# OmerShubi/DL_VQA

Measured on AMD Instinct MI355X. Metric: VQA samples/sec (train step), higher is better.
Workload: dtype f32; 1 GPU; VqaNet train step (fwd+softCE+bwd+Adam), batch 256/GPU, 224x224 images, 14-token questions, 1000-way head, train mode; global_batch=256, image_size=224, answers=1000, vocab=5000, parallelism=dp1

## Files before the change

dl_vqa_amd/_lib.py:

```python
from __future__ import annotations

import ctypes as C
import os

import torch

_HERE = os.path.dirname(os.path.abspath(__file__))
LIB_PATH = os.environ.get("VQA_LIB", os.path.join(_HERE, "libvqa_hip.so"))
HEADER_PATH = os.path.join(os.path.dirname(_HERE), "include", "vqa_hip.h")


def header_abi_version() -> int:
    import re
    with open(HEADER_PATH) as f:
        m = re.search(r"^#define\s+VQA_ABI_VERSION\s+(\d+)", f.read(), flags=re.M)
    if not m:
        raise VqaHipError(f"{HEADER_PATH}: no VQA_ABI_VERSION")
    return int(m.group(1))


f32p = C.c_void_p
u8p = C.c_void_p
i64p = C.c_void_p
i32, i64, f32, u64, vp = C.c_int, C.c_int64, C.c_float, C.c_uint64, C.c_void_p
# ... 96 lines not shown
    "vqa_gemm_tall_bf16_supported": (i32, [i32, i32, i32, i32, i32]),
    "vqa_gemm_tall_bf16_plan": (i32, [i32, i32, i32, C.POINTER(i32), i32]),
    "vqa_gemm_tall_bf16": (i32, [vp, i64, vp, i64, vp, i64, i32, i32, i32, f32p, i64, i32, i32, i32, i32, vp]),
    "vqa_conv_pack_weights_bf16": (i32, [f32p, vp, vp, i32, i32, i32, vp]),
    "vqa_conv3x3_relu_pool_fwd_bf16": (i32, [vp, vp, f32p, vp, i32, u8p, i32, i32, i32, i32, i32, i32, i32, vp]),
    "vqa_conv3x3_dgrad_bf16": (i32, [vp, u8p, vp, vp, i32, i32, i32, i32, i32, i32, i32, i32, vp]),
    "vqa_conv3x3_wgrad_bf16_workspace_bytes": (i64, [i32, i32, i32, i32, i32, i32]),
    "vqa_conv3x3_wgrad_bf16": (i32, [vp, vp, u8p, f32p, f32p, i32, i32, i32, i32, i32, i32, i32, f32p, i64, i32, vp]),
    "vqa_pconvf_supported": (i32, [i32, i32, i32, i32, i32]),
    "vqa_pconvf_weights_bytes": (i64, [i32, i32]),
    "vqa_pconvf_pack_weights": (i32, [f32p, f32p, i32, i32, vp]),
    "vqa_pconvf_dgrad": (i32, [f32p, u8p, f32p, f32p, i32, i32, i32, i32, i32, i32, vp]),
    "vqa_pconv_supported": (i32, [i32, i32, i32, i32, i32]),
    "vqa_pconv_weights_bytes": (i64, [i32, i32]),
    "vqa_pconv_pack_weights": (i32, [f32p, vp, vp, i32, i32, vp]),
    "vqa_pconv_fwd": (i32, [vp, vp, f32p, vp, i32, u8p, i32, i32, i32, i32, i32, i32, vp]),
    "vqa_pconv_wgrad_supported": (i32, [i32, i32, i32, i32]),
    "vqa_pconv_wgrad_workspace_bytes": (i64, [i32, i32, i32, i32, i32]),
    "vqa_pconv_wgrad": (i32, [vp, u8p, vp, f32p, f32p, i32, i32, i32, i32, i32, f32p, i64, i32, vp]),
    "vqa_pconv_dgrad": (i32, [vp, u8p, vp, vp, i32, i32, i32, i32, i32, i32, i32, vp]),
    "vqa_adam": (i32, [f32p, f32p, f32p, f32p, i64, f32, f32, f32, f32, i32, f32, vp]),
    "vqa_adam_segments": (i32, [f32p, f32p, f32p, f32p, i64, vp, i32, f32, vp]),
    "vqa_conv3x3_x3_plan": (i32, [i32, i32, i32, i32, i32, i32, i32, C.POINTER(i32), i32]),
}

K_GEMM, K_CONV_FWD, K_CONV_DGRAD, K_CONV_WGRAD = 0, 1, 2, 3
(K_L2NORM_FWD, K_L2NORM_BWD, K_ATT_SCORE_FWD, K_ATT_SCORE_BWD, K_ATT_APPLY_FWD, K_ATT_APPLY_BWD, K_ADAM, K_SOFTCE,
 K_DROPOUT, K_LSTM_SEQ, K_COUNT) = range(4, 15)


class LstmDir(C.Structure):
    _fields_ = [("w_hh", vp), ("xg", vp), ("gates", vp), ("Hs", vp), ("Cs", vp), ("c_final", vp),
                ("dgates", vp), ("dh", vp), ("dc", vp), ("reverse", i32)]


class AdamSegment(C.Structure):
    _fields_ = [("begin", i64), ("end", i64), ("lr", f32), ("beta1", f32), ("beta2", f32), ("eps", f32),
                ("weight_decay", f32), ("step", i32), ("decoupled", i32)]


ADAM_MAX_SEGMENTS = 64


class VqaHipError(RuntimeError):
    pass


_lib = None


def load() -> C.CDLL:
    global _lib
    if _lib is not None:
        return _lib
    if not os.path.exists(LIB_PATH):
        raise VqaHipError(
            f"{LIB_PATH} not found: build it with `python -m dl_vqa_amd.build` "
            "(the HIP extension is mandatory; there is no CPU fallback)")
    lib = C.CDLL(LIB_PATH)
    for name, (res, args) in PROTOTYPES.items():
        fn = getattr(lib, name)
        fn.restype = res
        fn.argtypes = args
    want = header_abi_version()
# ... 21 lines not shown
```

dl_vqa_amd/build.py:

```python
from __future__ import annotations

import os
import subprocess
import sys
from concurrent.futures import ThreadPoolExecutor

HERE = os.path.dirname(os.path.abspath(__file__))
CSRC = os.path.join(HERE, "csrc")
LIB = os.path.join(HERE, "libvqa_hip.so")
SOURCES = ([("gemm.hip", f"_p{k}", [f"-DVQA_GEMM_PART={k}"]) for k in (2, 3, 4, 5)]
           + [("gemm_x3.hip", f"_p{k}", [f"-DVQA_GEMM_PART={k}"]) for k in (1, 2, 3, 4)]
           + ["bf16.hip", ("gemm.hip", "_p1", ["-DVQA_GEMM_PART=1"]), "conv.hip", "conv_x3.hip", "conv_bf16.hip", "conv_patch_bf16.hip", "conv_patch_f32.hip", "gemm_tall_bf16.hip", "gemm.hip",
              "gemm_x3.hip", "runtime.hip", "conv0.hip", "conv0_dgrad.hip", "lstm.hip", "elementwise.hip", "conv_generic.hip", "att_score.hip", "topk.hip", "preprocess.hip"])
HEADERS = ["common.hpp", "gemm_core.hpp", "gemm_epilogue.hpp", "gemm_host.hpp", "bf16_core.hpp", "x3_core.hpp", "conv_device.inc", "conv_host.inc", "conv_bf16.inc", os.path.join("..", "..", "include", "vqa_hip.h")]
FLAGS = ["-O3", "--offload-arch=gfx950", "-fPIC", "-std=c++17", "-Wno-unused-result"]


def _hipcc() -> str:
    for cand in (os.environ.get("HIPCC"), "/opt/rocm/bin/hipcc", "hipcc"):
        if cand and (os.path.isabs(cand) and os.path.exists(cand) or not os.path.isabs(cand)):
            return cand
    return "hipcc"


def _stale(target: str, deps) -> bool:
    if not os.path.exists(target):
        return True
    t = os.path.getmtime(target)
    return any(os.path.getmtime(d) > t for d in deps if os.path.exists(d))


def _deps(src: str, seen=None) -> list:
    import re
    seen = set() if seen is None else seen
    out = []
# ... 45 lines not shown
```

dl_vqa_amd/csrc/common.hpp:

```cpp
#pragma once
#include <hip/hip_runtime.h>
#include <stdint.h>
#include <stdio.h>
#include <string.h>

#include <type_traits>

#include "../../include/vqa_hip.h"

namespace vqa {

void set_error(const char* fmt, ...);
int check_hip(hipError_t e, const char* what);

#define VQA_REQUIRE(cond, ...)                 \
  do {                                         \
    if (!(cond)) {                             \
      ::vqa::set_error(__VA_ARGS__);           \
      return VQA_ERR_INVALID;                  \
    }                                          \
  } while (0)

int ensure_dyn_smem(const void* kernel, int bytes, const char* what);
template <class K>
// ... 27 lines not shown
  return with_flag(a, [&](auto fa) { return with_flag(b, [&](auto fb) { return f(fa, fb); }); });
}
template <class F>
static int with_int14(int v, F&& f) {
  switch (v) {
    case 1: return f(std::integral_constant<int, 1>{});
    case 2: return f(std::integral_constant<int, 2>{});
    case 3: return f(std::integral_constant<int, 3>{});
    default: return f(std::integral_constant<int, 4>{});
  }
}

static inline float keep_scale(float p) { return p > 0.f ? 1.0f / (1.0f - p) : 1.0f; }

struct Knobs {
  int split_target;
  int big_tiles;
  int persistent;
  int weight_stationary;
  int wgrad_192;
  int wgrad_384;
  int conv_chunk;
  int tall_bm;
};
const Knobs& knobs();

void set_launch_tag(int tag);
struct ProfScope {
  int id;
  hipStream_t s;
  bool on;
  ProfScope(int id_, hipStream_t s_);
  ~ProfScope();
};

__device__ __forceinline__ int xcd_swizzle(int bid, int nwg) {
  const int xcd = bid & 7, q = nwg >> 3, r = nwg & 7;
  const int base = (xcd < r) ? xcd * (q + 1) : r * (q + 1) + (xcd - r) * q;
  return base + (bid >> 3);
}

__device__ __forceinline__ uint32_t mix32(uint32_t x) {
  x ^= x >> 16; x *= 0x7feb352dU; x ^= x >> 15; x *= 0x846ca68bU; x ^= x >> 16;
  return x;
}
__device__ __forceinline__ uint32_t drop_hash(uint64_t seed, uint64_t pair) {
// ... 48 lines not shown
```

dl_vqa_amd/csrc/runtime.hip:

```cpp
#include <stdarg.h>
#include <stdlib.h>

#include <map>
#include <mutex>
#include <set>
#include <utility>
#include <vector>

#include "gemm_host.hpp"

namespace vqa {

static thread_local char g_err[512] = "";
void set_error(const char* fmt, ...) {
  va_list ap;
  va_start(ap, fmt);
  vsnprintf(g_err, sizeof(g_err), fmt, ap);
  va_end(ap);
}
int check_hip(hipError_t e, const char* what) {
  if (e == hipSuccess) return VQA_OK;
  set_error("%s: %s", what, hipGetErrorString(e));
  return VQA_ERR_HIP;
}
// ... 41 lines not shown
    return -1;
  }
  const int slots = cus * (per_cu < planned_per_cu ? per_cu : planned_per_cu);
  cache[key] = slots;
  return slots;
}

static std::mutex g_knob_mu;
static Knobs g_knobs;
static bool g_knobs_read = false;
static int env_int(const char* name) {
  const char* e = getenv(name);
  return (e && *e) ? atoi(e) : -1;
}
static void read_knobs_locked() {
  g_knobs.split_target = env_int("VQA_SPLIT_TARGET");
  g_knobs.big_tiles = env_int("VQA_BIG_TILES");
  g_knobs.persistent = env_int("VQA_PERSISTENT");
  g_knobs.weight_stationary = env_int("VQA_WEIGHT_STATIONARY");
  g_knobs.wgrad_192 = env_int("VQA_WGRAD_192");
  g_knobs.wgrad_384 = env_int("VQA_WGRAD_384");
  g_knobs.conv_chunk = env_int("VQA_CONV_CHUNK");
  g_knobs.tall_bm = env_int("VQA_TALL_BM");
  g_knobs_read = true;
}
const Knobs& knobs() {
  std::lock_guard<std::mutex> lk(g_knob_mu);
  if (!g_knobs_read) read_knobs_locked();
  return g_knobs;
}

static std::mutex g_prof_mu;
static uint32_t g_prof_mask = 0;
static int g_prof_tag = -1;
static std::vector<std::pair<hipEvent_t, hipEvent_t>> g_prof_ev;
static std::vector<std::pair<int, int>> g_prof_key;
static thread_local int g_launch_tag = -1;
void set_launch_tag(int tag) { g_launch_tag = tag; }

ProfScope::ProfScope(int id_, hipStream_t s_) : id(id_), s(s_), on(false) {
  if (g_prof_mask == 0) return;
  std::lock_guard<std::mutex> lk(g_prof_mu);
  if (!((g_prof_mask >> id) & 1u) || (g_prof_tag >= 0 && g_prof_tag != g_launch_tag)) return;
  hipStreamCaptureStatus cap = hipStreamCaptureStatusNone;
  if (hipStreamIsCapturing(s, &cap) != hipSuccess || cap != hipStreamCaptureStatusNone) return;
  hipEvent_t a, b;
// ... 152 lines not shown
```

dl_vqa_amd/engine.py:

```python
from __future__ import annotations

import functools
import inspect
import os
from collections import namedtuple
from types import SimpleNamespace
from typing import Callable, Dict, Optional

import torch

from . import ops

Tensor = torch.Tensor

SITE_IMAGE, SITE_TEXT, SITE_ATT_V, SITE_ATT_Q, SITE_ATT_X, SITE_CLS1, SITE_CLS2 = 1, 2, 3, 4, 5, 6, 7
_MASK64 = (1 << 64) - 1


def _site_seed(base: int, site: int) -> int:
    return (base * 0x9E3779B97F4A7C15 + site * 0xD1B54A32D192ED03 + 0x632BE59BD9B4E019) & _MASK64


_SFX = ("", "_reverse")

ConvRoute = namedtuple("ConvRoute", "kind x_shape Co src out dy dx x3 pdg pack_in need_wd")
_OUT16 = {"nhwc32": torch.float32, "nhwc16": torch.bfloat16, "c16": torch.bfloat16}


def _gemm(A, B, C, M, N, K, x3=False, **kw):
    if A.dtype == torch.bfloat16:
        assert not x3
        return ops.gemm_bf16(A, B, C, M, N, K, **kw)
    return ops.gemm(A, B, C, M, N, K, x3=x3, **kw)


def _device_current(name: str, device=lambda x: x.device):
    def deco(schedule):
        pos = list(inspect.signature(schedule).parameters).index(name) - 1

        @functools.wraps(schedule)
        def guarded(self, *args, **kw):
            with torch.cuda.device(device(args[pos] if pos < len(args) else kw[name])):
                return schedule(self, *args, **kw)
        return guarded
    return deco

# ... 31 lines not shown
        self.GC = self.G * self.C
        self.Dc = self.GC + self.Q
        for name, val in (("embedding_features", self.E), ("question_features", self.H), ("hidden_dim(att)", self.mid),
                          ("hidden_dim(cls)", self.hid)) + tuple((f"num_channels[{k}]", ch) for k, ch in
                                                                 enumerate(self.channels[1:], 1)):
            if val % 4:
                raise ValueError(f"{name}={val}: the HIP kernels need multiples of 4 (16-byte vector loads)")
        if self.channels[0] > 4:
            raise ValueError("input images with more than 4 channels are not supported")
        if compute_dtype not in ("fp32", "bf16", "fp32x3"):
            raise ValueError(f"compute_dtype {compute_dtype!r} (fp32, fp32x3 or bf16)")
        if self.ks != 3 and compute_dtype != "fp32":
            raise ValueError(f"compute_dtype {compute_dtype!r} needs image.kernel_size=3 (kernel_size={self.ks} runs in fp32)")
        self.bf16 = compute_dtype == "bf16"
        self.x3 = compute_dtype == "fp32x3"
        self.x3_gemm = self.x3 and os.environ.get("VQA_X3_GEMM", "1") != "0"
        self.fc16 = (self.bf16 and os.environ.get("VQA_FC16", "1") != "0"
                     and all(d % 8 == 0 for d in (self.Q, self.mid, self.Dc, self.hid, self.A)))
        self.lstm16 = self.bf16 and os.environ.get("VQA_LSTM16", "1") != "0" and self.H % 8 == 0
        if self.bf16:
            if self.L < 2 or any(ch % 64 for ch in self.channels[1:]) or self.mid % 8 or self.stride != 1:
                raise ValueError("the bf16 path needs >= 2 conv blocks, stride 1 and channel counts that are multiples "
                                 f"of 64 after the first block (num_channels={self.channels}, stride={self.stride})")
        self._sides = {}

    def conv_routes(self, v_shape, keep: bool, need_dx: bool = False):
        B, C, H, W = v_shape
        L, ch, bf16 = self.L, self.channels, self.bf16
        fast0 = self.ks == 3 and ops.conv0_supported(C, H, W, ch[1], self.stride)
        if bf16 and not fast0:
            raise ValueError("the bf16 path needs the dedicated first-block kernel (3-channel NCHW image, "
                             "W % 4 == 0, 32 or 64 output channels)")
        shapes = [(B, H, W, C if fast0 else 4)]
        for l in range(1, L):
            H, W = ops.convk_out_hw(H, W, self.ks, self.stride)[2:]
            shapes.append((B, H, W, ch[l]))
        use_pc = bf16 and os.environ.get("VQA_PCONV", "1") != "0" and all(
            ops.pconv_supported(h, w, ci, co, 1) and ci % 64 == 0 and ops.pconv_wgrad_supported(h, w, ci, co)
            for (_, h, w, ci), co in zip(shapes[1:], ch[2:]))
        kinds = ["convk" if self.ks != 3 else "conv0" if l == 0 and fast0 else
                 ("pconv" if use_pc else "conv16") if bf16 else "conv32" for l in range(L)]
        x3 = [k == "conv32" and self._x3_layer(s, co) for k, s, co in zip(kinds, shapes, ch[1:])] + [False]
        pdg_mode = os.environ.get("VQA_PDGRAD", "1")
        routes = []
        for l, (kind, s) in enumerate(zip(kinds, shapes)):
            last, src = l == L - 1, routes[-1].out if l else "nchw" if fast0 else "nhwc32"
# ... 112 lines not shown
        q_len = q_len.to(device=dev, dtype=torch.int64).contiguous()
        x_emb = ops.embed_tanh_fwd(q, P["text.embedding.weight"], p_txt, _site_seed(seed, SITE_TEXT), bad_tokens)
        combined = torch.empty(q.shape[0], self.Dc, dtype=torch.float32, device=dev)
        encode = lambda: self._question_encoder(P, x_emb, q_len, combined, l16)
        (lstm, x16), done = self._on_side_stream(dev, encode) if side else (encode(), None)
        return SimpleNamespace(q=q, q_len=q_len, x_emb=x_emb, combined=combined, lstm=lstm, x16=x16), done

    @staticmethod
    def _saved(txt, qlin, cls, seed, rates, Pn, vn, v_in, vprime, score, probs, pooled=None, **own):
        (qp, q_in, ld_q, fc), (c_in, h1, h1d), (p_txt, p_att, p_cls) = qlin, cls, rates
        B, T = txt.q.shape
        stages = dict(score=score, combined=txt.combined)
        if pooled is not None:
            stages["pooled"] = pooled
        return SimpleNamespace(B=B, T=T, Pn=Pn, q=txt.q, q_len=txt.q_len, x_emb=txt.x_emb, x16=txt.x16, lstm=txt.lstm, vn=vn,
                               v_in=v_in, vprime=vprime, qp=qp, q_in=q_in, ld_q=ld_q, fc=fc, probs=probs, c_in=c_in, h1=h1,
                               h1d=h1d, p_txt=p_txt, p_att=p_att, p_cls=p_cls, seed=seed, stages=stages, **own)

    @staticmethod
    def _encoder_saved(enc, norm, p_img, need_dx, v):
        return dict(routes=enc.routes, acts=enc.acts, idxs=enc.idxs, wds=enc.wds, norm=norm, fast0=enc.fast0, use_pc=enc.use_pc,
                    p_img=p_img, need_dx=need_dx, v_dtype=v.dtype, v_shape=tuple(v.shape))

    def _question_encoder(self, P, x_emb, q_len, combined, l16):
        T, B, E = x_emb.shape
        H, Dc, GC = self.H, self.Dc, self.GC
        new = lambda *shape: torch.empty(*shape, dtype=torch.float32, device=x_emb.device)
        Ek = (E + 7) // 8 * 8 if l16 else E
        x16 = self._cols16(x_emb, T * B, E, Ek) if l16 else None
        lstm = []
        for d in range(self.ndir):
            xg = new(T * B, 4 * H)
            w_ih = P["text.lstm.weight_ih_l0" + _SFX[d]]
            wih16 = self._cols16(w_ih, 4 * H, E, Ek) if l16 else None
            _gemm(x16 if l16 else x_emb, wih16 if l16 else w_ih, xg, T * B, 4 * H, Ek,
                  bias1=P["text.lstm.bias_ih_l0" + _SFX[d]], bias2=P["text.lstm.bias_hh_l0" + _SFX[d]], tag=10)
            st = dict(w_hh=P["text.lstm.weight_hh_l0" + _SFX[d]], xg=xg, gates=new(T, B, 4 * H), Hs=new(T + 1, B, H),
                      Cs=new(T + 1, B, H), c_final=combined[:, GC + d * H:], reverse=bool(d), wih16=wih16)
            st["Hs"][T if d else 0].zero_()
            st["Cs"][T if d else 0].zero_()
            lstm.append(st)
        fused, use_graph = self._lstm_schedule()
        if fused:
            ops.lstm_seq_fwd(lstm, q_len, B, T, H, cf_ld=Dc, use_graph=use_graph)
            return lstm, x16
        for st in lstm:
            hg = new(B, 4 * H)
            for n, (t, si, so) in enumerate(self._lstm_steps(T, st["reverse"])):
                ops.gemm(st["Hs"][si], st["w_hh"], hg, B, 4 * H, H, tag=11)
                ops.lstm_cell_fwd(st["xg"][t * B:(t + 1) * B], hg, st["Cs"][si], st["Hs"][si], q_len, t, st["gates"][t],
                                  st["Cs"][so], st["Hs"][so], st["c_final"] if n == T - 1 else None, Dc)
        return lstm, x16

    def _image_encoder(self, P, v, keep, need_dx=False):
        routes = self.conv_routes(tuple(v.shape), keep, need_dx)
        x = v
        if routes[0].src != "nchw":
            x = ops.nchw_to_nhwc4(ops.half_to_float(v) if v.dtype == torch.float16 else v)
        acts, idxs, wds = [], [], []
        for l, r in enumerate(routes):
            w, bias = P[f"image.conv{l}.weight"], P[f"image.conv{l}.bias"]
            assert w.shape[0] == r.Co
            x, y, am, wd = getattr(self, f"_{r.kind}_fwd")(r, l, x, w, bias)
            if keep:
# ... 344 lines not shown
        dev = dcomb.device
        new = lambda *shape: torch.empty(*shape, dtype=torch.float32, device=dev)
        dirs = []
        for d, st in enumerate(ctx.lstm):
            dc = new(B, H)
            ops.add2d(dcomb[:, GC + d * H:], Dc, None, 0, dc, H, B, H)
            dh = torch.zeros(B, H, dtype=torch.float32, device=dev)
            st["dgates"] = new(T, B, 4 * H)
            dirs.append(dict(w_hh=P["text.lstm.weight_hh_l0" + _SFX[d]], gates=st["gates"], Hs=st["Hs"], Cs=st["Cs"],
                             dgates=st["dgates"], dh=dh, dc=dc, reverse=bool(d)))
        fused, use_graph = self._lstm_schedule()
        if fused:
            ops.lstm_seq_bwd(dirs, ctx.q_len, B, T, H, use_graph=use_graph)
        else:
            for st in dirs:
                for n, (t, si, so) in enumerate(reversed(self._lstm_steps(T, st["reverse"]))):
                    ops.lstm_cell_bwd(st["gates"][t], st["Cs"][si], st["Cs"][so], ctx.q_len, t, st["dh"], st["dc"],
                                      st["dgates"][t])
                    if n != T - 1:
                        ops.gemm(st["dgates"][t], st["w_hh"], st["dh"], B, H, 4 * H, transB=False, lda=4 * H, ldb=H,
                                 accumulate=True, tag=50)
        l16 = ctx.x16 is not None
        x_op, Ek = (ctx.x16, ctx.x16.shape[1]) if l16 else (ctx.x_emb, E)
        dx_parts = []
        for d, st in enumerate(ctx.lstm):
            dgates = st["dgates"]
            h_in = st["Hs"][0:T] if d == 0 else st["Hs"][1:T + 1]
            dw_hh, dw_ih, dx = Gr["text.lstm.weight_hh_l0" + _SFX[d]], Gr["text.lstm.weight_ih_l0" + _SFX[d]], new(T * B, E)
            if l16:
                dg_op, h_op, wih_op = ops.to_bf16(dgates.view(T * B, 4 * H)), ops.to_bf16(h_in.reshape(T * B, H)), st["wih16"]
            else:
                dg_op, h_op, wih_op = dgates, h_in, P["text.lstm.weight_ih_l0" + _SFX[d]]
            _gemm(dg_op, h_op, dw_hh, 4 * H, H, T * B, transA=True, transB=False, lda=4 * H, ldb=H, tag=51)
            dwp = dw_ih if Ek == E else new(4 * H, Ek)
            _gemm(dg_op, x_op, dwp, 4 * H, Ek, T * B, transA=True, transB=False, lda=4 * H, ldb=Ek, tag=52)
            if Ek != E:
                ops.add2d(dwp, Ek, None, 0, dw_ih, E, 4 * H, E)
            ops.colsum(dgates, T * B, 4 * H, Gr["text.lstm.bias_ih_l0" + _SFX[d]])
            ops.add2d(Gr["text.lstm.bias_ih_l0" + _SFX[d]], 4 * H, None, 0, Gr["text.lstm.bias_hh_l0" + _SFX[d]], 4 * H, 1, 4 * H)
            dxp = dx if Ek == E else new(T * B, Ek)
            _gemm(dg_op, wih_op, dxp, T * B, Ek, 4 * H, transB=False, lda=4 * H, ldb=Ek, tag=53)
            if Ek != E:
                ops.add2d(dxp, Ek, None, 0, dx, E, T * B, E)
            dx_parts.append(dx)
        dx_emb = dx_parts[0]
        if self.ndir > 1:
            ops.add(dx_parts[0], dx_parts[1], dx_emb)
        ops.embed_tanh_bwd(ctx.q, ctx.x_emb, dx_emb, Gr["text.embedding.weight"], ctx.p_txt, _site_seed(ctx.seed, SITE_TEXT))

    def _image_bwd(self, P, ctx, dcomb, dv_in, Gr):
        sd = lambda site: _site_seed(ctx.seed, site)
        c16_hw = tuple(ctx.idxs[-1].shape[2:4]) if ctx.routes[-1].dy == "c16" else None
        dP = ops.l2norm_bwd_joined(dcomb, self.Dc, ctx.probs, dv_in, ctx.p_att, sd(SITE_ATT_V), ctx.vn, ctx.norm, ctx.p_img,
                                   sd(SITE_IMAGE), out_dtype=torch.bfloat16 if self.bf16 else torch.float32, c16_hw=c16_hw)
        if c16_hw is None:
            dP = dP.view_as(ctx.acts[-1])
        return self._conv_bwd(P, ctx, dP, Gr)

    def _conv_bwd(self, P, ctx, dP, Gr):
        for l, r in reversed(list(enumerate(ctx.routes))):
            dP = getattr(self, f"_{r.kind}_bwd")(r, l, ctx, dP, Gr[f"image.conv{l}.weight"], Gr[f"image.conv{l}.bias"],
                                                 P[f"image.conv{l}.weight"])
        if ctx.routes[0].dx == "nhwc32":
            return ops.nhwc_to_nchw(dP, ctx.v_shape[1], out_dtype=ctx.v_dtype)
        return dP

    def _convk_bwd(self, r, l, ctx, dP, dw, db, w):
# ... 23 lines not shown
```

dl_vqa_amd/ops.py:

```python
from __future__ import annotations

from typing import Optional, Tuple

import torch

from . import _lib
from ._lib import call, ptr, stream

_ws = {}


def workspace(nbytes: int, device) -> torch.Tensor:
    key = (str(device), torch.cuda.current_stream(device).cuda_stream)
    t = _ws.get(key)
    if t is None or t.numel() * 4 < nbytes:
        t = torch.empty(_workspace_floats(nbytes), dtype=torch.float32, device=device)
        _ws[key] = t
    return t


def _workspace_floats(nbytes: int) -> int:
    return max(nbytes // 4 + 1024, 1 << 20)


# ... 16 lines not shown
    return C


def gemm(A: torch.Tensor, B: torch.Tensor, C: torch.Tensor, M: int, N: int, K: int, *, transA=False,
         transB=True, lda=None, ldb=None, ldc=None, bias1=None, bias2=None, rowgroup=None, rg_div=1,
         rg_op=0, relu=False, accumulate=False, aux=None, tag=0, x3=False) -> torch.Tensor:
    return _gemm("vqa_gemm_x3" if x3 else "vqa_gemm", (), A, B, C, M, N, K, transA, transB, lda, ldb, ldc, bias1, bias2, rowgroup,
                 rg_div, rg_op, relu, accumulate, aux, tag)


GEMM_ENGINES = {"vqa_gemm": 0, "vqa_gemm_x3": 1, "vqa_gemm_bf16": 2}
GEMM_PLAN_FIELDS = ("BM", "BN", "tiles_m", "tiles_n", "nk", "splits", "ks_per_split", "order", "persistent", "wide")


def gemm_plan(engine: str, M: int, N: int, K: int, *, transA=False, transB=True, workspace_bytes=None) -> dict:
    import ctypes
    lib = _lib.load()
    if workspace_bytes is None:
        nbytes = getattr(lib, engine + "_workspace_bytes")(M, N, K) if min(M, N, K) > 0 else 0
        workspace_bytes = _workspace_floats(nbytes) * 4 if nbytes else 0
    out = (ctypes.c_int32 * len(GEMM_PLAN_FIELDS))()
    call("vqa_gemm_plan", GEMM_ENGINES[engine], M, N, K, int(transA), int(transB), workspace_bytes, out, len(out))
    return dict(zip(GEMM_PLAN_FIELDS, out))


def nchw_to_nhwc4(x: torch.Tensor) -> torch.Tensor:
    B, Cc, H, W = x.shape
    y = torch.empty(B, H, W, 4, dtype=torch.float32, device=x.device)
    call("vqa_nchw_to_nhwc4", ptr(x), ptr(y), B, Cc, H, W, stream())
    return y


def conv_pack_weights(w: torch.Tensor, CiP: int, need_wd: bool = True):
    Co, Ci = w.shape[0], w.shape[1]
    wf = torch.empty(9 * CiP, Co, dtype=torch.float32, device=w.device)
    wd = torch.empty(9 * Co, CiP, dtype=torch.float32, device=w.device) if need_wd else None
    call("vqa_conv_pack_weights", ptr(w), ptr(wf), ptr(wd), Co, Ci, CiP, stream())
    return wf, wd


def conv_out_hw(H: int, W: int, stride: int) -> Tuple[int, int]:
    return ((H - 3) // stride + 1) // 2, ((W - 3) // stride + 1) // 2


def convk_out_hw(H: int, W: int, ks: int, stride: int) -> Tuple[int, int, int, int]:
    Ho, Wo = (H - ks) // stride + 1, (W - ks) // stride + 1
# ... 810 lines not shown
```

include/vqa_hip.h:

```cpp
#ifndef VQA_HIP_H
#define VQA_HIP_H

#include <stdint.h>

#ifdef __cplusplus
extern "C" {
#endif

#define VQA_ABI_VERSION 9

#define VQA_OK 0
#define VQA_ERR_INVALID 1
#define VQA_ERR_HIP 2
#define VQA_ERR_WORKSPACE 3

typedef void* vqa_stream_t;

int vqa_abi_version(void);
const char* vqa_last_error(void);
int vqa_device_ok(void);

int vqa_reload_knobs(void);

enum {
// ... 251 lines not shown
int64_t vqa_gemm_x3_workspace_bytes(int M, int N, int K);
int vqa_gemm_x3(const float* A, int64_t lda, int transA, const float* B, int64_t ldb, int transB, float* C, int64_t ldc,
                int M, int N, int K, const float* bias1, const float* bias2, const float* rowgroup, int64_t rg_ld,
                int rg_div, int rg_op, int relu, int accumulate, float* aux, float* workspace, int64_t workspace_bytes,
                int tag, vqa_stream_t stream);

int vqa_adam(float* param, const float* grad, float* exp_avg, float* exp_avg_sq, int64_t n, float lr,
             float beta1, float beta2, float eps, int step, float grad_scale, vqa_stream_t stream);

#define VQA_ADAM_MAX_SEGMENTS 64
#define VQA_ADAM_SEGMENTS_MAX_BLOCKS 2048
typedef struct {
  int64_t begin, end;
  float lr, beta1, beta2, eps, weight_decay;
  int step;
  int decoupled;
} vqa_adam_segment;
int vqa_adam_segments(float* param, const float* grad, float* exp_avg, float* exp_avg_sq, int64_t n,
                      const vqa_adam_segment* segs , int n_segs, float grad_scale,
                      vqa_stream_t stream);

int vqa_conv3x3_x3_plan(int pass, int B, int H, int W, int CiP, int Co, int stride, int32_t* out, int n_out);

#ifdef __cplusplus
}
#endif
#endif
```

Baseline: 9955 samples/s.

## Add grouped GEMM kernel to batch the two LSTM directions' GEMMs into one launch

Adds a grouped f32 GEMM (up to 4 same-shape problems in one launch, with split-K and persistent variants plus a grouped split-K reduce). The bidirectional LSTM's input projection and its backward dw_hh, dw_ih and dx GEMMs now run as one grouped launch per kind instead of one launch per direction. The aim is to cut launch count and fill the GPU better on these small GEMMs. The cost is a separate planner whose tile and split choices may suit some shapes worse than the tuned single GEMM path.

```diff
diff --git a/dl_vqa_amd/_lib.py b/dl_vqa_amd/_lib.py
--- a/dl_vqa_amd/_lib.py
+++ b/dl_vqa_amd/_lib.py
@@ -142,6 +142,9 @@
     "vqa_adam": (i32, [f32p, f32p, f32p, f32p, i64, f32, f32, f32, f32, i32, f32, vp]),
     "vqa_adam_segments": (i32, [f32p, f32p, f32p, f32p, i64, vp, i32, f32, vp]),
     "vqa_conv3x3_x3_plan": (i32, [i32, i32, i32, i32, i32, i32, i32, C.POINTER(i32), i32]),
+    "vqa_gemm_grouped_workspace_bytes": (i64, [i32, i32, i32, i32]),
+    "vqa_gemm_grouped_plan": (i32, [i32, i32, i32, i32, C.POINTER(i32), i32]),
+    "vqa_gemm_grouped": (i32, [vp, i32, i32, i32, i32, i32, i32, i32, f32p, i64, i32, vp]),
 }
 
 K_GEMM, K_CONV_FWD, K_CONV_DGRAD, K_CONV_WGRAD = 0, 1, 2, 3
@@ -160,6 +163,13 @@
 
 
 ADAM_MAX_SEGMENTS = 64
+
+
+class GemmProblem(C.Structure):
+    _fields_ = [("A", vp), ("lda", i64), ("B", vp), ("ldb", i64), ("C", vp), ("ldc", i64), ("bias1", vp), ("bias2", vp)]
+
+
+GEMM_GROUP_MAX = 4
 
 
 class VqaHipError(RuntimeError):
diff --git a/dl_vqa_amd/build.py b/dl_vqa_amd/build.py
--- a/dl_vqa_amd/build.py
+++ b/dl_vqa_amd/build.py
@@ -10,7 +10,8 @@
 LIB = os.path.join(HERE, "libvqa_hip.so")
 SOURCES = ([("gemm.hip", f"_p{k}", [f"-DVQA_GEMM_PART={k}"]) for k in (2, 3, 4, 5)]
            + [("gemm_x3.hip", f"_p{k}", [f"-DVQA_GEMM_PART={k}"]) for k in (1, 2, 3, 4)]
-           + ["bf16.hip", ("gemm.hip", "_p1", ["-DVQA_GEMM_PART=1"]), "conv.hip", "conv_x3.hip", "conv_bf16.hip", "conv_patch_bf16.hip", "conv_patch_f32.hip", "gemm_tall_bf16.hip", "gemm.hip",
+           + [("gemm_grouped.hip", f"_p{k}", [f"-DVQA_GEMM_PART={k}"]) for k in (1, 2, 3, 4)]
+           + ["bf16.hip", ("gemm.hip", "_p1", ["-DVQA_GEMM_PART=1"]), "gemm_grouped.hip", "conv.hip", "conv_x3.hip", "conv_bf16.hip", "conv_patch_bf16.hip", "conv_patch_f32.hip", "gemm_tall_bf16.hip", "gemm.hip",
               "gemm_x3.hip", "runtime.hip", "conv0.hip", "conv0_dgrad.hip", "lstm.hip", "elementwise.hip", "conv_generic.hip", "att_score.hip", "topk.hip", "preprocess.hip"])
 HEADERS = ["common.hpp", "gemm_core.hpp", "gemm_epilogue.hpp", "gemm_host.hpp", "bf16_core.hpp", "x3_core.hpp", "conv_device.inc", "conv_host.inc", "conv_bf16.inc", os.path.join("..", "..", "include", "vqa_hip.h")]
 FLAGS = ["-O3", "--offload-arch=gfx950", "-fPIC", "-std=c++17", "-Wno-unused-result"]
diff --git a/dl_vqa_amd/csrc/common.hpp b/dl_vqa_amd/csrc/common.hpp
--- a/dl_vqa_amd/csrc/common.hpp
+++ b/dl_vqa_amd/csrc/common.hpp
@@ -73,6 +73,8 @@
   int wgrad_384;
   int conv_chunk;
   int tall_bm;
+  int grouped_splits;
+  int grouped_wide;
 };
 const Knobs& knobs();
 
diff --git a/dl_vqa_amd/csrc/gemm_grouped.hip b/dl_vqa_amd/csrc/gemm_grouped.hip
--- /dev/null
+++ b/dl_vqa_amd/csrc/gemm_grouped.hip
@@ -0,0 +1,264 @@
+#include "gemm_host.hpp"
+
+#ifndef VQA_GEMM_PART
+#define VQA_GEMM_PART 0
+#endif
+
+namespace vqa {
+
+using CfgG128 = TileCfg<128, 128, 2, 2>;
+using CfgGWide = TileCfg<128, 320, 4, 2>;
+constexpr int GROUPED_WIDE_BN = CfgGWide::BN;
+constexpr int GROUPED_SLOTS_128 = 512, GROUPED_SLOTS_WIDE = 256;
+
+struct GroupedArgs {
+  const float* A[VQA_GEMM_GROUP_MAX]; const float* B[VQA_GEMM_GROUP_MAX]; float* C[VQA_GEMM_GROUP_MAX];
+  const float* bias1[VQA_GEMM_GROUP_MAX]; const float* bias2[VQA_GEMM_GROUP_MAX];
+  int64_t lda[VQA_GEMM_GROUP_MAX], ldb[VQA_GEMM_GROUP_MAX], ldc[VQA_GEMM_GROUP_MAX];
+  int n, M, N, K, accumulate;
+  float* slab;
+};
+
+struct GroupedPlan { GemmPlan g; int n, wide, persistent, grid; };
+GroupedPlan plan_gemm_grouped(int n, int M, int N, int K);
+
+__device__ __forceinline__ EpiParams grouped_epi(const GroupedArgs& g, int prob) {
+  EpiParams pe{};
+  pe.C = g.C[prob]; pe.ldc = g.ldc[prob]; pe.M = g.M; pe.N = g.N;
+  pe.bias1 = g.bias1[prob]; pe.bias2 = g.bias2[prob];
+  pe.rg_div = 1; pe.accumulate = g.accumulate;
+  return pe;
+}
+
+template <class Cfg, class AL, class BL>
+int launch_gemm_grouped(const GroupedArgs& g, const GroupedPlan& p, hipStream_t s);
+
+#if VQA_GEMM_PART != 0
+struct GroupedCoord { int prob, mt, nt, split; };
+__device__ __forceinline__ GroupedCoord grouped_coord(int t, int tiles_m, int tiles_n, int splits) {
+  const int tiles = tiles_m * tiles_n, per = tiles * splits;
+  GroupedCoord c;
+  c.prob = t / per;
+  const int u = t - c.prob * per;
+  c.split = u / tiles;
+  const int v = u - c.split * tiles;
+  c.mt = v / tiles_n;
+  c.nt = v - c.mt * tiles_n;
+  return c;
+}
+
+template <class Cfg>
+__device__ __forceinline__ void grouped_epilogue(const EpiParams& pe, f32x16 (&acc)[Cfg::TM][Cfg::TN], int m0, int n0, int wm,
+                                                 int wn, int lane) {
+  if (pe.accumulate) gemm_epilogue_mode<Cfg, 0, true, false>(pe, acc, m0, n0, wm, wn, lane);
+  else gemm_epilogue_mode<Cfg, 0, false, false>(pe, acc, m0, n0, wm, wn, lane);
+}
+
+template <class Cfg, class AL, class BL>
+__global__ __launch_bounds__(Cfg::THREADS, Cfg::MIN_WAVES) void gemm_grouped_kernel(GroupedArgs g, int tiles_m, int tiles_n, int nk,
+                                                                                      int ks_per_split, int splits) {
+  extern __shared__ __attribute__((aligned(16))) float smem[];
+  const int tid = threadIdx.x, lane = tid & 63, wave = tid >> 6;
+  const int wm = wave / Cfg::WAVES_N, wn = wave % Cfg::WAVES_N;
+  const GroupedCoord tc = grouped_coord(xcd_swizzle(blockIdx.x, gridDim.x), tiles_m, tiles_n, splits);
+  const int m0 = tc.mt * Cfg::BM, n0 = tc.nt * Cfg::BN;
+  const int ks0 = tc.split * ks_per_split;
+  const int ks1 = min(nk, ks0 + ks_per_split);
+  f32x16 acc[Cfg::TM][Cfg::TN];
+  acc_zero<Cfg>(acc);
+  if (!gemm_mainloop<Cfg, AL, BL>(
+          [&](AL& al, BL& bl) {
+            al.init({g.A[tc.prob], g.lda[tc.prob], g.M, g.K}, m0, loader_tid<Cfg>(), ks0);
+            bl.init({g.B[tc.prob], g.ldb[tc.prob], g.N, g.K}, n0, loader_tid<Cfg>(), ks0);
+          },
+          [](AL&, BL&) {}, acc, ks0, ks1, g.K, smem))
+    return;
+  if (g.slab) {
+    float* slab = g.slab + ((int64_t)tc.split * g.n + tc.prob) * g.M * g.N;
+    store_acc_tiles<Cfg>(acc, slab, g.N, g.M, g.N, m0, n0, wm, wn, lane);
+    return;
+  }
+  grouped_epilogue<Cfg>(grouped_epi(g, tc.prob), acc, m0, n0, wm, wn, lane);
+}
+
+template <class Cfg, class AL, class BL>
+__global__ __launch_bounds__(Cfg::THREADS, Cfg::MIN_WAVES) void gemm_grouped_persistent_kernel(GroupedArgs g, int tiles_m, int tiles_n,
+                                                                                                 int nk) {
+  extern __shared__ __attribute__((aligned(16))) float smem[];
+  const int lane = threadIdx.x & 63, wave = threadIdx.x >> 6;
+  const int wm = wave / Cfg::WAVES_N, wn = wave % Cfg::WAVES_N;
+  gemm_persistent<Cfg, AL, BL, false>(
+      xcd_swizzle(blockIdx.x, gridDim.x), gridDim.x, g.n * tiles_m * tiles_n, nk, g.K, smem,
+      [&](int t, AL& al, BL& bl) {
+        const GroupedCoord tc = grouped_coord(t, tiles_m, tiles_n, 1);
+        al.init({g.A[tc.prob], g.lda[tc.prob], g.M, g.K}, tc.mt * Cfg::BM, loader_tid<Cfg>(), 0);
+        bl.init({g.B[tc.prob], g.ldb[tc.prob], g.N, g.K}, tc.nt * Cfg::BN, loader_tid<Cfg>(), 0);
+      },
+      [&](int t, f32x16 (&acc)[Cfg::TM][Cfg::TN]) {
+        const GroupedCoord tc = grouped_coord(t, tiles_m, tiles_n, 1);
+        grouped_epilogue<Cfg>(grouped_epi(g, tc.prob), acc, tc.mt * Cfg::BM, tc.nt * Cfg::BN, wm, wn, lane);
+      });
+}
+
+template <class Cfg, class AL, class BL>
+int launch_gemm_grouped(const GroupedArgs& g, const GroupedPlan& p, hipStream_t s) {
+  using SL = SmemLayout<Cfg, AL::kTypeR, BL::kTypeR>;
+  const int tiles = p.n * p.g.tiles_m * p.g.tiles_n;
+  if constexpr (SL::WG_PER_CU == 2) {
+    if (p.persistent) {
+      auto pk = gemm_grouped_persistent_kernel<Cfg, AL, BL>;
+      if (int rc = ensure_dyn_smem(reinterpret_cast<const void*>(pk), SL::BYTES, "hipFuncSetAttribute(gemm_grouped_persistent)")) return rc;
+      const int slots = persistent_slots(reinterpret_cast<const void*>(pk), Cfg::THREADS, SL::BYTES, SL::WG_PER_CU);
+      if (slots <= 0) return VQA_ERR_HIP;
+      hipLaunchKernelGGL(pk, dim3(tiles < slots ? tiles : slots), dim3(Cfg::THREADS), SL::BYTES, s, g, p.g.tiles_m, p.g.tiles_n, p.g.nk);
+      return check_hip(hipGetLastError(), "gemm_grouped_persistent_kernel launch");
+    }
+  }
+  if (p.persistent) { set_error("vqa_gemm_grouped: the plan asks for a persistent launch of a tile that has none"); return VQA_ERR_INVALID; }
+  auto kern = gemm_grouped_kernel<Cfg, AL, BL>;
+  if (int rc = ensure_dyn_smem(reinterpret_cast<const void*>(kern), SL::BYTES, "hipFuncSetAttribute(gemm_grouped)")) return rc;
+  hipLaunchKernelGGL(kern, dim3(tiles * p.g.splits), dim3(Cfg::THREADS), SL::BYTES, s, g, p.g.tiles_m, p.g.tiles_n, p.g.nk,
+                     p.g.ks_per_split, p.g.splits);
+  return check_hip(hipGetLastError(), "gemm_grouped_kernel launch");
+}
+
+#define VQA_GROUPED_OWN(CFG, AL, BL) \
+  template int launch_gemm_grouped<CFG, AL<CFG::NVA, CFG::LT>, BL<CFG::NVB, CFG::LT>>(const GroupedArgs&, const GroupedPlan&, hipStream_t);
+#if VQA_GEMM_PART == 1
+VQA_GROUPED_OWN(CfgG128, PlainR, PlainR) VQA_GROUPED_OWN(CfgG128, PlainR, PlainC)
+#elif VQA_GEMM_PART == 2
+VQA_GROUPED_OWN(CfgG128, PlainC, PlainC)
+#elif VQA_GEMM_PART == 3
+VQA_GROUPED_OWN(CfgGWide, PlainR, PlainR) VQA_GROUPED_OWN(CfgGWide, PlainR, PlainC)
+#elif VQA_GEMM_PART == 4
+VQA_GROUPED_OWN(CfgGWide, PlainC, PlainC)
+#endif
+
+}
+
+#else
+GroupedPlan plan_gemm_grouped(int n, int M, int N, int K) {
+  const Knobs& kn = knobs();
+  GroupedPlan p{};
+  p.n = n;
+  const int wide_tm = (M + CfgGWide::BM - 1) / CfgGWide::BM;
+  p.wide = N > 256 && N <= GROUPED_WIDE_BN && n * wide_tm <= GROUPED_SLOTS_WIDE && kn.grouped_wide != 0;
+  const int bm = p.wide ? CfgGWide::BM : CfgG128::BM, bn = p.wide ? CfgGWide::BN : CfgG128::BN;
+  const int slots = p.wide ? GROUPED_SLOTS_WIDE : GROUPED_SLOTS_128;
+  p.g.big = 1;
+  p.g.tiles_m = (M + bm - 1) / bm;
+  p.g.tiles_n = (N + bn - 1) / bn;
+  p.g.nk = (K + BK - 1) / BK;
+  const int64_t tiles = (int64_t)n * p.g.tiles_m * p.g.tiles_n;
+  int splits = 1;
+  if (tiles < slots) {
+    const int fill = (int)(slots / tiles), deep = p.g.nk / 16 > 1 ? p.g.nk / 16 : 1;
+    splits = kn.grouped_splits > 0 ? kn.grouped_splits : (fill < deep ? fill : deep);
+    if (splits > fill) splits = fill;
+    if (splits > 64) splits = 64;
+  }
+  split_k(p.g, splits);
+  p.persistent = !p.wide && p.g.splits == 1 && (p.g.nk <= 16 || tiles > slots);
+  p.grid = p.persistent ? (int)(tiles < slots ? tiles : slots) : (int)tiles * p.g.splits;
+  return p;
+}
+
+template <bool VEC>
+__global__ __launch_bounds__(256) void splitk_reduce_grouped_kernel(GroupedArgs g, int splits) {
+  const int prob = blockIdx.y;
+  const EpiParams pe = grouped_epi(g, prob);
+  constexpr int W = VEC ? 4 : 1;
+  const int64_t total = (int64_t)g.M * g.N / W, per_split = (int64_t)g.n * total;
+  const int nw = g.N / W;
+  for (int64_t e = (int64_t)blockIdx.x * blockDim.x + threadIdx.x; e < total; e += (int64_t)gridDim.x * blockDim.x) {
+    float r[W];
+#pragma unroll
+    for (int k = 0; k < W; ++k) r[k] = 0.f;
+#pragma unroll 4
+    for (int sp = 0; sp < splits; ++sp) {
+      const int64_t at = sp * per_split + prob * total + e;
+      if constexpr (VEC) {
+        const float4 a = reinterpret_cast<const float4*>(g.slab)[at];
+        r[0] += a.x; r[1] += a.y; r[2] += a.z; r[3] += a.w;
+      } else {
+        r[0] += g.slab[at];
+      }
+    }
+    const int row = (int)(e / nw), col = W * (int)(e - (int64_t)row * nw);
+#pragma unroll
+    for (int k = 0; k < W; ++k) pe.C[(int64_t)row * pe.ldc + col + k] = epi_apply(pe, r[k], row, col + k);
+  }
+}
+
+static int launch_splitk_reduce_grouped(const GroupedArgs& g, int splits, hipStream_t s) {
+  const bool vec = g.N % 4 == 0;
+  const int64_t total = (int64_t)g.M * g.N / (vec ? 4 : 1);
+  const dim3 grid(grid_for(total, 256, 2048), g.n);
+  if (vec) hipLaunchKernelGGL(splitk_reduce_grouped_kernel<true>, grid, dim3(256), 0, s, g, splits);
+  else hipLaunchKernelGGL(splitk_reduce_grouped_kernel<false>, grid, dim3(256), 0, s, g, splits);
+  return check_hip(hipGetLastError(), "splitk_reduce_grouped launch");
+}
+
+template <class Cfg>
+static int dispatch_gemm_grouped(int transA, int transB, const GroupedArgs& g, const GroupedPlan& p, hipStream_t s) {
+  using AR = PlainR<Cfg::NVA, Cfg::LT>; using AC = PlainC<Cfg::NVA, Cfg::LT>;
+  using BR = PlainR<Cfg::NVB, Cfg::LT>; using BC = PlainC<Cfg::NVB, Cfg::LT>;
+  if (transA) return launch_gemm_grouped<Cfg, AC, BC>(g, p, s);
+  return transB ? launch_gemm_grouped<Cfg, AR, BR>(g, p, s) : launch_gemm_grouped<Cfg, AR, BC>(g, p, s);
+}
+
+static int check_grouped_shape(const char* name, int n, int M, int N, int K) {
+  VQA_REQUIRE(n >= 1 && n <= VQA_GEMM_GROUP_MAX, "%s: n=%d problems (1..%d)", name, n, VQA_GEMM_GROUP_MAX);
+  VQA_REQUIRE(M > 0 && N > 0 && K > 0, "%s: bad shape M=%d N=%d K=%d", name, M, N, K);
+  return VQA_OK;
+}
+
+}
+
+using namespace vqa;
+
+extern "C" {
+
+int64_t vqa_gemm_grouped_workspace_bytes(int n, int M, int N, int K) {
+  if (check_grouped_shape("vqa_gemm_grouped_workspace_bytes", n, M, N, K)) return 0;
+  return slab_bytes(plan_gemm_grouped(n, M, N, K).g, n * M, N);
+}
+
+int vqa_gemm_grouped_plan(int n, int M, int N, int K, int32_t* out, int n_out) {
+  if (int rc = check_grouped_shape("vqa_gemm_grouped_plan", n, M, N, K)) return rc;
+  VQA_REQUIRE(out && n_out >= 9, "vqa_gemm_grouped_plan: out needs 9 entries (n_out=%d)", n_out);
+  const GroupedPlan p = plan_gemm_grouped(n, M, N, K);
+  const int32_t v[9] = {p.wide ? CfgGWide::BM : CfgG128::BM, p.wide ? CfgGWide::BN : CfgG128::BN, p.g.tiles_m, p.g.tiles_n, p.g.nk,
+                        p.g.splits, p.g.ks_per_split, p.grid, p.persistent};
+  for (int i = 0; i < 9; ++i) out[i] = v[i];
+  return VQA_OK;
+}
+
+int vqa_gemm_grouped(const vqa_gemm_problem* problems, int n, int transA, int transB, int M, int N, int K, int accumulate,
+                     float* workspace, int64_t workspace_bytes, int tag, vqa_stream_t stream) {
+  if (int rc = check_grouped_shape("vqa_gemm_grouped", n, M, N, K)) return rc;
+  VQA_REQUIRE(problems, "vqa_gemm_grouped: null problem table");
+  VQA_REQUIRE(!(transA && transB), "vqa_gemm_grouped: A stored [K][M] with B stored [N][K] is not built");
+  GroupedArgs g{};
+  for (int i = 0; i < n; ++i) {
+    const vqa_gemm_problem& q = problems[i];
+    if (int rc = check_gemm_args("vqa_gemm_grouped", 4, q.A, q.lda, q.B, q.ldb, q.C, q.ldc, M, N, K, nullptr, 1)) return rc;
+    g.A[i] = q.A; g.B[i] = q.B; g.C[i] = q.C; g.bias1[i] = q.bias1; g.bias2[i] = q.bias2;
+    g.lda[i] = q.lda; g.ldb[i] = q.ldb; g.ldc[i] = q.ldc;
+  }
+  g.n = n; g.M = M; g.N = N; g.K = K; g.accumulate = accumulate;
+  hipStream_t s = (hipStream_t)stream;
+  const GroupedPlan p = plan_gemm_grouped(n, M, N, K);
+  EpiParams slabs{};
+  slabs.M = n * M; slabs.N = N;
+  if (int rc = claim_slab("vqa_gemm_grouped", p.g, slabs, workspace, workspace_bytes)) return rc;
+  g.slab = slabs.slab;
+  set_launch_tag(tag);
+  ProfScope prof(VQA_K_GEMM, s);
+  int rc = p.wide ? dispatch_gemm_grouped<CfgGWide>(transA, transB, g, p, s) : dispatch_gemm_grouped<CfgG128>(transA, transB, g, p, s);
+  if (rc == 0 && p.g.splits > 1) rc = launch_splitk_reduce_grouped(g, p.g.splits, s);
+  return rc;
+}
+
+}
+#endif
diff --git a/dl_vqa_amd/csrc/runtime.hip b/dl_vqa_amd/csrc/runtime.hip
--- a/dl_vqa_amd/csrc/runtime.hip
+++ b/dl_vqa_amd/csrc/runtime.hip
@@ -87,6 +87,8 @@
   g_knobs.wgrad_384 = env_int("VQA_WGRAD_384");
   g_knobs.conv_chunk = env_int("VQA_CONV_CHUNK");
   g_knobs.tall_bm = env_int("VQA_TALL_BM");
+  g_knobs.grouped_splits = env_int("VQA_GROUPED_SPLITS");
+  g_knobs.grouped_wide = env_int("VQA_GROUPED_WIDE");
   g_knobs_read = true;
 }
 const Knobs& knobs() {
diff --git a/dl_vqa_amd/engine.py b/dl_vqa_amd/engine.py
--- a/dl_vqa_amd/engine.py
+++ b/dl_vqa_amd/engine.py
@@ -22,6 +22,8 @@
 
 
 _SFX = ("", "_reverse")
+LSTM_GROUPED_ALL = ("xg", "dw_hh", "dw_ih", "dx")
+LSTM_GROUPED = ("xg", "dw_hh", "dw_ih", "dx")
 
 ConvRoute = namedtuple("ConvRoute", "kind x_shape Co src out dy dx x3 pdg pack_in need_wd")
 _OUT16 = {"nhwc32": torch.float32, "nhwc16": torch.bfloat16, "c16": torch.bfloat16}
@@ -99,6 +101,8 @@
             if self.L < 2 or any(ch % 64 for ch in self.channels[1:]) or self.mid % 8 or self.stride != 1:
                 raise ValueError("the bf16 path needs >= 2 conv blocks, stride 1 and channel counts that are multiples "
                                  f"of 64 after the first block (num_channels={self.channels}, stride={self.stride})")
+        self.lstm_grouped = frozenset(filter(None, os.environ.get("VQA_LSTM_GROUPED", ",".join(LSTM_GROUPED)).split(",")))
+        assert self.lstm_grouped <= set(LSTM_GROUPED_ALL), self.lstm_grouped
         self._sides = {}
 
     def conv_routes(self, v_shape, keep: bool, need_dx: bool = False):
@@ -257,6 +261,9 @@
         return dict(routes=enc.routes, acts=enc.acts, idxs=enc.idxs, wds=enc.wds, norm=norm, fast0=enc.fast0, use_pc=enc.use_pc,
                     p_img=p_img, need_dx=need_dx, v_dtype=v.dtype, v_shape=tuple(v.shape))
 
+    def _lstm_pairs(self, l16):
+        return self.lstm_grouped if self.ndir == 2 and not l16 else frozenset()
+
     def _question_encoder(self, P, x_emb, q_len, combined, l16):
         T, B, E = x_emb.shape
         H, Dc, GC = self.H, self.Dc, self.GC
@@ -264,17 +271,26 @@
         Ek = (E + 7) // 8 * 8 if l16 else E
         x16 = self._cols16(x_emb, T * B, E, Ek) if l16 else None
         lstm = []
+        pair = self._lstm_pairs(l16)
+        if "xg" in pair and ops.gemm_plan("vqa_gemm", T * B, 4 * H, E)["splits"] != 1:
+            pair = pair - {"xg"}
+        xg_pair = []
         for d in range(self.ndir):
             xg = new(T * B, 4 * H)
             w_ih = P["text.lstm.weight_ih_l0" + _SFX[d]]
             wih16 = self._cols16(w_ih, 4 * H, E, Ek) if l16 else None
-            _gemm(x16 if l16 else x_emb, wih16 if l16 else w_ih, xg, T * B, 4 * H, Ek,
-                  bias1=P["text.lstm.bias_ih_l0" + _SFX[d]], bias2=P["text.lstm.bias_hh_l0" + _SFX[d]], tag=10)
+            biases = dict(bias1=P["text.lstm.bias_ih_l0" + _SFX[d]], bias2=P["text.lstm.bias_hh_l0" + _SFX[d]])
+            if "xg" in pair:
+                xg_pair.append(dict(A=x_emb, B=w_ih, C=xg, **biases))
+            else:
+                _gemm(x16 if l16 else x_emb, wih16 if l16 else w_ih, xg, T * B, 4 * H, Ek, tag=10, **biases)
             st = dict(w_hh=P["text.lstm.weight_hh_l0" + _SFX[d]], xg=xg, gates=new(T, B, 4 * H), Hs=new(T + 1, B, H),
                       Cs=new(T + 1, B, H), c_final=combined[:, GC + d * H:], reverse=bool(d), wih16=wih16)
             st["Hs"][T if d else 0].zero_()
             st["Cs"][T if d else 0].zero_()
             lstm.append(st)
+        if xg_pair:
+            ops.gemm_grouped(xg_pair, T * B, 4 * H, E, tag=10)
         fused, use_graph = self._lstm_schedule()
         if fused:
             ops.lstm_seq_fwd(lstm, q_len, B, T, H, cf_ld=Dc, use_graph=use_graph)
@@ -665,6 +681,8 @@
                                  accumulate=True, tag=50)
         l16 = ctx.x16 is not None
         x_op, Ek = (ctx.x16, ctx.x16.shape[1]) if l16 else (ctx.x_emb, E)
+        pair = self._lstm_pairs(l16)
+        grouped = {"dw_hh": [], "dw_ih": [], "dx": []}
         dx_parts = []
         for d, st in enumerate(ctx.lstm):
             dgates = st["dgates"]
@@ -674,18 +692,33 @@
                 dg_op, h_op, wih_op = ops.to_bf16(dgates.view(T * B, 4 * H)), ops.to_bf16(h_in.reshape(T * B, H)), st["wih16"]
             else:
                 dg_op, h_op, wih_op = dgates, h_in, P["text.lstm.weight_ih_l0" + _SFX[d]]
-            _gemm(dg_op, h_op, dw_hh, 4 * H, H, T * B, transA=True, transB=False, lda=4 * H, ldb=H, tag=51)
+            if "dw_hh" in pair:
+                grouped["dw_hh"].append(dict(A=dg_op, B=h_op, C=dw_hh))
+            else:
+                _gemm(dg_op, h_op, dw_hh, 4 * H, H, T * B, transA=True, transB=False, lda=4 * H, ldb=H, tag=51)
             dwp = dw_ih if Ek == E else new(4 * H, Ek)
-            _gemm(dg_op, x_op, dwp, 4 * H, Ek, T * B, transA=True, transB=False, lda=4 * H, ldb=Ek, tag=52)
+            if "dw_ih" in pair:
+                grouped["dw_ih"].append(dict(A=dg_op, B=x_op, C=dwp))
+            else:
+                _gemm(dg_op, x_op, dwp, 4 * H, Ek, T * B, transA=True, transB=False, lda=4 * H, ldb=Ek, tag=52)
             if Ek != E:
                 ops.add2d(dwp, Ek, None, 0, dw_ih, E, 4 * H, E)
             ops.colsum(dgates, T * B, 4 * H, Gr["text.lstm.bias_ih_l0" + _SFX[d]])
             ops.add2d(Gr["text.lstm.bias_ih_l0" + _SFX[d]], 4 * H, None, 0, Gr["text.lstm.bias_hh_l0" + _SFX[d]], 4 * H, 1, 4 * H)
             dxp = dx if Ek == E else new(T * B, Ek)
-            _gemm(dg_op, wih_op, dxp, T * B, Ek, 4 * H, transB=False, lda=4 * H, ldb=Ek, tag=53)
+            if "dx" in pair:
+                grouped["dx"].append(dict(A=dg_op, B=wih_op, C=dxp))
+            else:
+                _gemm(dg_op, wih_op, dxp, T * B, Ek, 4 * H, transB=False, lda=4 * H, ldb=Ek, tag=53)
             if Ek != E:
                 ops.add2d(dxp, Ek, None, 0, dx, E, T * B, E)
             dx_parts.append(dx)
+        if grouped["dw_hh"]:
+            ops.gemm_grouped(grouped["dw_hh"], 4 * H, H, T * B, transA=True, transB=False, tag=51)
+        if grouped["dw_ih"]:
+            ops.gemm_grouped(grouped["dw_ih"], 4 * H, E, T * B, transA=True, transB=False, tag=52)
+        if grouped["dx"]:
+            ops.gemm_grouped(grouped["dx"], T * B, E, 4 * H, transB=False, tag=53)
         dx_emb = dx_parts[0]
         if self.ndir > 1:
             ops.add(dx_parts[0], dx_parts[1], dx_emb)
diff --git a/dl_vqa_amd/ops.py b/dl_vqa_amd/ops.py
--- a/dl_vqa_amd/ops.py
+++ b/dl_vqa_amd/ops.py
@@ -62,6 +62,32 @@
     out = (ctypes.c_int32 * len(GEMM_PLAN_FIELDS))()
     call("vqa_gemm_plan", GEMM_ENGINES[engine], M, N, K, int(transA), int(transB), workspace_bytes, out, len(out))
     return dict(zip(GEMM_PLAN_FIELDS, out))
+
+
+GEMM_GROUPED_PLAN_FIELDS = ("BM", "BN", "tiles_m", "tiles_n", "nk", "splits", "ks_per_split", "grid", "persistent")
+
+
+def gemm_grouped(problems, M: int, N: int, K: int, *, transA=False, transB=True, accumulate=False, tag=0) -> None:
+    lib = _lib.load()
+    n = len(problems)
+    table = (_lib.GemmProblem * max(n, 1))()
+    for t, p in zip(table, problems):
+        t.A, t.B, t.C = ptr(p["A"]), ptr(p["B"]), ptr(p["C"])
+        t.lda = p.get("lda") or (M if transA else K)
+        t.ldb = p.get("ldb") or (K if transB else N)
+        t.ldc = p.get("ldc") or N
+        t.bias1, t.bias2 = ptr(p.get("bias1")), ptr(p.get("bias2"))
+    nbytes = lib.vqa_gemm_grouped_workspace_bytes(n, M, N, K)
+    ws = workspace(nbytes, problems[0]["A"].device) if nbytes else None
+    call("vqa_gemm_grouped", table, n, int(transA), int(transB), M, N, K, int(accumulate), ptr(ws),
+         (ws.numel() * 4 if ws is not None else 0), tag, stream())
+
+
+def gemm_grouped_plan(n: int, M: int, N: int, K: int) -> dict:
+    import ctypes
+    out = (ctypes.c_int32 * len(GEMM_GROUPED_PLAN_FIELDS))()
+    call("vqa_gemm_grouped_plan", n, M, N, K, out, len(out))
+    return dict(zip(GEMM_GROUPED_PLAN_FIELDS, out))
 
 
 def nchw_to_nhwc4(x: torch.Tensor) -> torch.Tensor:
diff --git a/include/vqa_hip.h b/include/vqa_hip.h
--- a/include/vqa_hip.h
+++ b/include/vqa_hip.h
@@ -297,6 +297,19 @@
 
 int vqa_conv3x3_x3_plan(int pass, int B, int H, int W, int CiP, int Co, int stride, int32_t* out, int n_out);
 
+#define VQA_GEMM_GROUP_MAX 4
+typedef struct {
+  const float* A; int64_t lda;
+  const float* B; int64_t ldb;
+  float* C; int64_t ldc;
+  const float* bias1;
+  const float* bias2;
+} vqa_gemm_problem;
+int64_t vqa_gemm_grouped_workspace_bytes(int n, int M, int N, int K);
+int vqa_gemm_grouped_plan(int n, int M, int N, int K, int32_t* out, int n_out);
+int vqa_gemm_grouped(const vqa_gemm_problem* problems , int n, int transA, int transB, int M, int N, int K,
+                     int accumulate, float* workspace, int64_t workspace_bytes, int tag, vqa_stream_t stream);
+
 #ifdef __cplusplus
 }
 #endif
```

Result: no change. 10030 samples/s (median of 6 runs) (+0.8%).
